# NTT123/vietTTS

Hardware: NVIDIA B200
Metric: audio_samples_per_sec (higher is better)
Workload: dtype f32 (bf16x3 split products on tcgen05, fp32 accumulate/storage)

## Files before the change

### viettts_b200/csrc/nat.cu

```cuda
#include <cooperative_groups.h>

#include "vtts_internal.cuh"

namespace cg = cooperative_groups;

namespace {

constexpr int SCAN_CTAS = 128;
constexpr int SCAN_THREADS = 256;
constexpr int UPC = 4;
constexpr int NCOL = 16;
constexpr int RG = 8;
constexpr int NSLICE = 64;
constexpr int MAX_ROWS = 128;

__device__ __forceinline__ float sigmoidf_(float x) { return 1.f / (1.f + expf(-x)); }

__host__ __device__ inline void threefry2x32(uint32_t k0, uint32_t k1, uint32_t c0, uint32_t c1, uint32_t& o0, uint32_t& o1) {
  const uint32_t ks2 = 0x1BD11BDAu ^ k0 ^ k1;
  uint32_t x0 = c0 + k0, x1 = c1 + k1;
  const int R0[4] = {13, 15, 26, 6}, R1[4] = {17, 29, 16, 24};
  const uint32_t ks[3] = {k0, k1, ks2};
#pragma unroll
  for (int blk = 0; blk < 5; ++blk) {
// ... 109 lines not shown
      acc[f][0] = fmaf(ww, x.x, acc[f][0]);
      acc[f][1] = fmaf(ww, x.y, acc[f][1]);
    }
  }
#pragma unroll
  for (int f = 0; f < UP_F; ++f) {
    const int n = f0 + f;
    if (n < nf) {
      float2 o = make_float2(acc[f][0], acc[f][1]);
      *reinterpret_cast<float2*>(out + ((size_t)b * N + n) * out_ld + tid * 2) = o;
    }
  }
}

struct Seg {
  const float* p;
  int n;
  int stride;
};

__device__ __forceinline__ float lstm_cell(const float* zs, int r, int uu, float zadd_i, float zadd_g, float zadd_f, float zadd_o, float& c) {
  const float zi = zs[r * NCOL + 0 * UPC + uu] + zadd_i;
  const float zg = zs[r * NCOL + 1 * UPC + uu] + zadd_g;
  const float zf = zs[r * NCOL + 2 * UPC + uu] + zadd_f;
  const float zo = zs[r * NCOL + 3 * UPC + uu] + zadd_o;
  const float f = sigmoidf_(zf + 1.f);
  c = f * c + sigmoidf_(zi) * tanhf(zg);
  return sigmoidf_(zo) * tanhf(c);
}

struct EncScanArgs {
  const float* zx;
  const float* whr;
  const int32_t* lengths;
  float* out;
  int B, L;
};

struct DecScanArgs {
  const float* zc0;
  const float* zc1;
  const float* w0r;
  const float* w1r;
  const float* wc;
  const float* bc;
  const float* wp2;
  const uint8_t* keep;
  uint64_t seed;
  int mode;
  float* p1;
  float* p2;
  float* h0;
  float* h1;
  unsigned int* pre_bar;
  int* err;
  float* hout;
  int B, N;
  int row_base;
  int N_total_rows;
  long long* dbg;
};

constexpr int DEC_XR = 32;
constexpr int DEC_NG = 4;
constexpr int DEC_KPAD = vc::PRENET + 2 * vc::DEC_H + 4;
constexpr int DEC_LSTM = 128, DEC_PRE = 16;
constexpr int DEC_CTAS = DEC_LSTM + DEC_PRE;

__device__ __forceinline__ void dec_fetch(float* xs, int pitch, int koff, const float* p, int n, int stride, int nr) {
  const int n4 = n >> 2;
  const int total = nr * n4;
  for (int e0 = threadIdx.x; e0 < total; e0 += SCAN_THREADS * 8) {
    float4 v[8];
#pragma unroll
    for (int u = 0; u < 8; ++u) {
      const int e = e0 + u * SCAN_THREADS;
      v[u] = make_float4(0.f, 0.f, 0.f, 0.f);
      if (e < total && p) {
        const int r = e / n4, i4 = (e - r * n4) * 4;
        v[u] = __ldcg(reinterpret_cast<const float4*>(p + (size_t)r * stride + i4));
      }
    }
#pragma unroll
    for (int u = 0; u < 8; ++u) {
      const int e = e0 + u * SCAN_THREADS;
      if (e < total) {
        const int r = e / n4, i4 = (e - r * n4) * 4;
        *reinterpret_cast<float4*>(xs + (size_t)r * pitch + koff + i4) = v[u];
      }
    }
  }
}

__device__ __forceinline__ void dec_fetch_async(float* xs, int pitch, int koff, const float* p, int n, int stride, int nr) {
  const int n4 = n >> 2;
  const int total = nr * n4;
  for (int e = threadIdx.x; e < total; e += SCAN_THREADS) {
    const int r = e / n4, i4 = (e - r * n4) * 4;
    const uint32_t dst = (uint32_t)__cvta_generic_to_shared(xs + (size_t)r * pitch + koff + i4);
    asm volatile("cp.async.cg.shared.global [%0], [%1], 16;" ::"r"(dst), "l"(p + (size_t)r * stride + i4) : "memory");
  }
  asm volatile("cp.async.commit_group;" ::: "memory");
}
template <int N>
__device__ __forceinline__ void cp_async_wait() { asm volatile("cp.async.wait_group %0;" ::"n"(N) : "memory"); }

__device__ __forceinline__ float4 warp_reduce_rows(float (&acc)[RG][4], int lane) {
  const bool b4 = lane & 16, b3 = lane & 8, b2 = lane & 4;
  float a4[4][4];
#pragma unroll
  for (int r = 0; r < 4; ++r)
#pragma unroll
    for (int c = 0; c < 4; ++c) {
      const float send = b4 ? acc[r][c] : acc[r + 4][c];
      const float keep = b4 ? acc[r + 4][c] : acc[r][c];
      a4[r][c] = keep + __shfl_xor_sync(0xffffffffu, send, 16);
    }
  float a2[2][4];
#pragma unroll
  for (int r = 0; r < 2; ++r)
#pragma unroll
    for (int c = 0; c < 4; ++c) {
      const float send = b3 ? a4[r][c] : a4[r + 2][c];
      const float keep = b3 ? a4[r + 2][c] : a4[r][c];
      a2[r][c] = keep + __shfl_xor_sync(0xffffffffu, send, 8);
    }
  float a1[4];
#pragma unroll
  for (int c = 0; c < 4; ++c) {
    const float send = b2 ? a2[0][c] : a2[1][c];
    const float keep = b2 ? a2[1][c] : a2[0][c];
    a1[c] = keep + __shfl_xor_sync(0xffffffffu, send, 4);
  }
  return make_float4(a1[0], a1[1], a1[2], a1[3]);
}

template <int SL, int PITCH = DEC_KPAD>
__device__ __forceinline__ void dec_matmul(const float* __restrict__ xs, const float (&w)[SL][4], int ngroups, float* part, float* zout,
                                           const float* zadd) {
  const int tid = threadIdx.x, lane = tid & 31, warp = tid >> 5;
  const int ks = tid >> 2;
  for (int g = 0; g < ngroups; ++g) {
    float acc[RG][4];
#pragma unroll
    for (int r = 0; r < RG; ++r) acc[r][0] = acc[r][1] = acc[r][2] = acc[r][3] = 0.f;
// ... 165 lines not shown
        acc[i][4] = fmaf(x, wb.x, acc[i][4]); acc[i][5] = fmaf(x, wb.y, acc[i][5]);
        acc[i][6] = fmaf(x, wb.z, acc[i][6]); acc[i][7] = fmaf(x, wb.w, acc[i][7]);
      }
    }
  }
  const bool b4 = lane & 16, b3 = lane & 8, b2 = lane & 4;
  float a4[4][8];
#pragma unroll
  for (int i = 0; i < 4; ++i)
#pragma unroll
    for (int c = 0; c < 8; ++c) {
      const float send = b4 ? acc[i][c] : acc[i + 4][c];
      const float keep = b4 ? acc[i + 4][c] : acc[i][c];
      a4[i][c] = keep + __shfl_xor_sync(0xffffffffu, send, 16);
    }
  float a2[2][8];
#pragma unroll
  for (int i = 0; i < 2; ++i)
#pragma unroll
    for (int c = 0; c < 8; ++c) {
      const float send = b3 ? a4[i][c] : a4[i + 2][c];
      const float keep = b3 ? a4[i + 2][c] : a4[i][c];
      a2[i][c] = keep + __shfl_xor_sync(0xffffffffu, send, 8);
    }
  float a1[8];
#pragma unroll
  for (int c = 0; c < 8; ++c) {
    const float send = b2 ? a2[0][c] : a2[1][c];
    const float keep = b2 ? a2[1][c] : a2[0][c];
    a1[c] = keep + __shfl_xor_sync(0xffffffffu, send, 4);
  }
  const int row = rg + 4 * ((lane >> 2) & 7);
  float* pw = part + ((size_t)warp * 32 + row) * 8;
  *reinterpret_cast<float4*>(pw) = make_float4(a1[0], a1[1], a1[2], a1[3]);
  *reinterpret_cast<float4*>(pw + 4) = make_float4(a1[4], a1[5], a1[6], a1[7]);
  __syncthreads();
  {
    float sum = 0.f;
#pragma unroll
    for (int wv = 0; wv < SCAN_THREADS / 32; ++wv) sum += part[(size_t)wv * 256 + tid];
    outv[tid] = sum;
  }
  __syncthreads();
}

__device__ __forceinline__ void pre_load_w8(float* wsm, const float* g, int K, int SL, int ld, int c0) {
  for (int e = threadIdx.x; e < K * 2; e += SCAN_THREADS) {
    const int k = e >> 1, h = (e & 1) * 4;
    const float4 v = __ldg(reinterpret_cast<const float4*>(g + (size_t)k * ld + c0 + h));
    *reinterpret_cast<float4*>(wsm + (size_t)(k + k / SL) * 8 + h) = v;
  }
}

__device__ __forceinline__ void prenet_barrier(unsigned int* counter, unsigned int target, int* err) {
  __syncthreads();
  if (threadIdx.x == 0) {
    __threadfence();
    atomicAdd(counter, 1u);
    const long long t0 = clock64();
    unsigned int v;
    do {
      asm volatile("ld.acquire.gpu.global.u32 %0, [%1];" : "=r"(v) : "l"(counter) : "memory");
      if (v < target && clock64() - t0 > 4000000000LL) {
        if (err) *err = 77;
        __threadfence_system();
        asm volatile("trap;");
      }
    } while (v < target);
  }
  __syncthreads();
}

__global__ void __launch_bounds__(SCAN_THREADS, 1) decoder_scan_kernel(const DecScanArgs a) {
  cg::grid_group grid = cg::this_grid();
  extern __shared__ __align__(16) float sm[];
  constexpr int H = vc::DEC_H, K0 = vc::PRENET + H, K1 = vc::PRENET + 2 * H;
  const int c = blockIdx.x, tid = threadIdx.x;
  const int B = a.B, N = a.N;
  long long tm[8] = {0, 0, 0, 0, 0, 0, 0, 0};
  long long tq = clock64();
#define DEC_MARK(i) { const long long tn = clock64(); tm[i] += tn - tq; tq = tn; }

  if (c < DEC_LSTM) {
    float* xs = sm;
    float* part = xs + DEC_XR * DEC_KPAD;
    float* zs = part + 8 * DEC_XR * NCOL;
    float* zp0 = zs + DEC_XR * NCOL;
    float* zp1 = zp0 + DEC_NG * DEC_XR * NCOL;
    float* cst = zp1 + DEC_NG * DEC_XR * NCOL;
    const int ks = tid >> 2, cgp = tid & 3;
    constexpr int SLP = vc::PRENET / NSLICE, SLH = H / NSLICE;
    float w0p[SLP][4], w0h[SLH][4], w1p[SLP][4], w1h0[SLH][4], w1h1[SLH][4];
    {
      auto ld = [&](float (&dst)[4], const float* base, int row) {
        const float4 v = __ldg(reinterpret_cast<const float4*>(base + (size_t)row * NCOL + cgp * 4));
        dst[0] = v.x; dst[1] = v.y; dst[2] = v.z; dst[3] = v.w;
      };
      const float* g0 = a.w0r + (size_t)c * K0 * NCOL;
      const float* g1 = a.w1r + (size_t)c * K1 * NCOL;
#pragma unroll
      for (int i = 0; i < SLP; ++i) { ld(w0p[i], g0, ks * SLP + i); ld(w1p[i], g1, ks * SLP + i); }
#pragma unroll
      for (int i = 0; i < SLH; ++i) {
        ld(w0h[i], g0, vc::PRENET + ks * SLH + i);
        ld(w1h0[i], g1, vc::PRENET + ks * SLH + i);
        ld(w1h1[i], g1, vc::PRENET + H + ks * SLH + i);
      }
    }
    for (int e = tid; e < DEC_NG * 2 * DEC_XR * UPC; e += SCAN_THREADS) cst[e] = 0.f;
    for (int e = tid; e < DEC_NG * 2 * DEC_XR * NCOL; e += SCAN_THREADS) zp0[e] = 0.f;
    for (int e = tid; e < DEC_XR * DEC_KPAD; e += SCAN_THREADS) xs[e] = 0.f;
    __syncthreads();
    const int NG = (B + DEC_XR - 1) / DEC_XR;
    for (int t = 0; t < N; ++t) {
      if (t > 0) {
        for (int rg = 0; rg < NG; ++rg) {
          const int r0 = rg * DEC_XR, nb = min(DEC_XR, B - r0), ngroups = (nb + RG - 1) / RG;
          if (NG > 1) dec_fetch(xs, DEC_KPAD, vc::PRENET, a.h0 + ((size_t)((t - 1) & 1) * B + r0) * H, H, H, nb);
          dec_fetch(xs, DEC_KPAD, vc::PRENET + H, a.h1 + ((size_t)((t - 1) & 1) * B + r0) * H, H, H, nb);
          if (NG > 1) __syncthreads();
          dec_matmul<SLH>(xs + vc::PRENET, w0h, ngroups, part, zp0 + rg * DEC_XR * NCOL, nullptr);
          dec_matmul<SLH>(xs + vc::PRENET + H, w1h1, ngroups, part, zp1 + rg * DEC_XR * NCOL, nullptr);
        }
      }
      DEC_MARK(0)
      DEC_MARK(1)
      DEC_MARK(2)
      grid.sync();
      DEC_MARK(3)
      for (int rg = 0; rg < NG; ++rg) {
        const int r0 = rg * DEC_XR, nb = min(DEC_XR, B - r0), ngroups = (nb + RG - 1) / RG;
        dec_fetch(xs, DEC_KPAD, 0, a.p2 + (size_t)r0 * vc::PRENET, vc::PRENET, vc::PRENET, nb);
        __syncthreads();
        dec_matmul<SLP>(xs, w0p, ngroups, part, zs, zp0 + rg * DEC_XR * NCOL);
        if (tid < nb * UPC) {
          const int r = tid / UPC, uu = tid % UPC, rb = r0 + r;
          const float* zc = a.zc0 + ((size_t)rb * N + t) * (4 * H) + c * UPC + uu;
          float* cs = cst + (size_t)rg * 2 * DEC_XR * UPC;
          float cc = cs[r * UPC + uu];
          const float h = lstm_cell(zs, r, uu, __ldg(zc), __ldg(zc + H), __ldg(zc + 2 * H), __ldg(zc + 3 * H), cc);
          cs[r * UPC + uu] = cc;
          a.h0[((size_t)(t & 1) * B + rb) * H + c * UPC + uu] = h;
          a.hout[((size_t)rb * N + t) * 2 * H + c * UPC + uu] = h;
        }
        if (NG > 1) __syncthreads();
      }
      DEC_MARK(4)
      grid.sync();
      DEC_MARK(5)
      for (int rg = 0; rg < NG; ++rg) {
        const int r0 = rg * DEC_XR, nb = min(DEC_XR, B - r0), ngroups = (nb + RG - 1) / RG;
        if (NG > 1) dec_fetch(xs, DEC_KPAD, 0, a.p2 + (size_t)r0 * vc::PRENET, vc::PRENET, vc::PRENET, nb);
        dec_fetch(xs, DEC_KPAD, vc::PRENET, a.h0 + ((size_t)(t & 1) * B + r0) * H, H, H, nb);
        __syncthreads();
        dec_matmul2<SLP, SLH>(xs, w1p, xs + vc::PRENET, w1h0, ngroups, part, zs, zp1 + rg * DEC_XR * NCOL);
        if (tid < nb * UPC) {
          const int r = tid / UPC, uu = tid % UPC, rb = r0 + r;
          const float* zc = a.zc1 + ((size_t)rb * N + t) * (4 * H) + c * UPC + uu;
          float* cs = cst + (size_t)rg * 2 * DEC_XR * UPC;
          float cc = cs[(DEC_XR + r) * UPC + uu];
          const float h = lstm_cell(zs, r, uu, __ldg(zc), __ldg(zc + H), __ldg(zc + 2 * H), __ldg(zc + 3 * H), cc);
          cs[(DEC_XR + r) * UPC + uu] = cc;
          a.h1[((size_t)(t & 1) * B + rb) * H + c * UPC + uu] = h;
          a.hout[((size_t)rb * N + t) * 2 * H + H + c * UPC + uu] = h;
        }
        __syncthreads();
      }
      DEC_MARK(6)
      grid.sync();
      DEC_MARK(7)
    }
  } else if (c < DEC_LSTM + DEC_PRE) {
    const int q = c - DEC_LSTM;
    constexpr int XP = H + 4;
    constexpr int WCB = (2 * H + 2 * H / 8) * 8;
    constexpr int W2B = (vc::PRENET + NSLICE) * 8;
    float* xs = sm;
    float* wcs = xs + 32 * XP;
    float* w2s = wcs + 2 * WCB;
    float* part = w2s + 2 * W2B;
    float* outv = part + 8 * 256;
    float* pp1 = outv + 256;
    for (int hf = 0; hf < 2; ++hf) {
      pre_load_w8(wcs + (size_t)hf * WCB, a.wc + (size_t)q * 2 * H * 16, 2 * H, 8, 16, hf * 8);
      pre_load_w8(w2s + (size_t)hf * W2B, a.wp2 + (size_t)q * vc::PRENET * 16, vc::PRENET, 4, 16, hf * 8);
    }
    for (int e = tid; e < 32 * XP; e += SCAN_THREADS) xs[e] = 0.f;
    for (int e = tid; e < DEC_NG * 512; e += SCAN_THREADS) pp1[e] = 0.f;
    __syncthreads();
    const int orow = tid >> 3, ocol = tid & 7;
    constexpr int H1OFF = (H + H / 8) * 8;
    const int NG = (B + DEC_XR - 1) / DEC_XR;
    for (int t = 0; t < N; ++t) {
      if (t > 0) {
        for (int rg = 0; rg < NG; ++rg) {
          const int r0 = rg * DEC_XR, nb = min(DEC_XR, B - r0);
          if (NG > 1) __syncthreads();
          dec_fetch(xs, XP, 0, a.h1 + ((size_t)((t - 1) & 1) * B + r0) * H, H, H, nb);
          __syncthreads();
#pragma unroll 1
          for (int hf = 0; hf < 2; ++hf) {
            pre_gemm8<8>(xs, XP, wcs + (size_t)hf * WCB + H1OFF, part, outv);
            if (orow < nb) {
              const int u = q * 16 + hf * 8 + ocol;
              const float v = fmaxf(outv[tid] + pp1[rg * 512 + hf * 256 + tid] + __ldg(a.bc + u), 0.f);
              a.p1[(size_t)(r0 + orow) * vc::PRENET + u] = v * keep_scale(a.mode, a.keep, a.seed, a.row_base + r0 + orow, t, N, 0, u);
            }
          }
        }
      } else {
        for (int e = tid; e < B * 16; e += SCAN_THREADS) a.p1[(size_t)(e >> 4) * vc::PRENET + q * 16 + (e & 15)] = 0.f;
      }
      DEC_MARK(0)
      prenet_barrier(a.pre_bar, (unsigned)DEC_PRE * (unsigned)(t + 1), a.err);
      DEC_MARK(1)
      for (int rg = 0; rg < NG; ++rg) {
        const int r0 = rg * DEC_XR, nb = min(DEC_XR, B - r0);
        if (NG > 1) __syncthreads();
        dec_fetch(xs, XP, 0, a.p1 + (size_t)r0 * vc::PRENET, vc::PRENET, vc::PRENET, nb);
        __syncthreads();
#pragma unroll 1
        for (int hf = 0; hf < 2; ++hf) {
          pre_gemm8<4>(xs, XP, w2s + (size_t)hf * W2B, part, outv);
          if (orow < nb) {
            const int u = q * 16 + hf * 8 + ocol;
            const float v = fmaxf(outv[tid], 0.f);
            a.p2[(size_t)(r0 + orow) * vc::PRENET + u] = v * keep_scale(a.mode, a.keep, a.seed, a.row_base + r0 + orow, t, N, 1, u);
          }
        }
      }
      DEC_MARK(2)
      grid.sync();
      DEC_MARK(3)
      grid.sync();
      DEC_MARK(5)
      for (int rg = 0; rg < NG; ++rg) {
        const int r0 = rg * DEC_XR, nb = min(DEC_XR, B - r0);
        __syncthreads();
        dec_fetch(xs, XP, 0, a.h0 + ((size_t)(t & 1) * B + r0) * H, H, H, nb);
        __syncthreads();
#pragma unroll 1
        for (int hf = 0; hf < 2; ++hf) {
          pre_gemm8<8>(xs, XP, wcs + (size_t)hf * WCB, part, outv);
          pp1[rg * 512 + hf * 256 + tid] = outv[tid];
        }
      }
      __syncthreads();
      DEC_MARK(6)
      grid.sync();
      DEC_MARK(7)
    }
  }
#undef DEC_MARK
  if (a.dbg && tid == 0)
    for (int i = 0; i < 8; ++i) a.dbg[(size_t)blockIdx.x * 16 + i] = tm[i];
}

__global__ void precompose_kernel(const float* __restrict__ wo, const float* __restrict__ bo, const float* __restrict__ w1,
                                  float* __restrict__ wc, float* __restrict__ bc) {
  const int o = threadIdx.x;
  const int i = blockIdx.x;
  double s = 0.0;
  if (i < 2 * vc::DEC_H) {
    for (int m = 0; m < vc::MEL; ++m) s += (double)wo[(size_t)i * vc::MEL + m] * (double)w1[(size_t)m * vc::PRENET + o];
    wc[(size_t)i * vc::PRENET + o] = (float)s;
  } else {
    for (int m = 0; m < vc::MEL; ++m) s += (double)bo[m] * (double)w1[(size_t)m * vc::PRENET + o];
    bc[o] = (float)s;
  }
}

struct TfScanArgs {
  const float* zc0;
  const float* zc1;
  const float* w0r;
  const float* w1r;
  const uint8_t* zone;
  uint64_t seed;
  int mode;
  float* h0s;
  float* h1s;
  float* hout;
  int B, N;
  int row_base;
};

constexpr int TF_PITCH = 3 * vc::DEC_H + 4;

__device__ __forceinline__ bool zone_keep(int mode, const uint8_t* zone, uint64_t seed, int b, int t, int N, int which, int unit) {
  if (mode == VTTS_DROPOUT_OFF) return false;
  if (mode == VTTS_DROPOUT_MASK) return zone[(((size_t)b * N + t) * 4 + which) * vc::DEC_H + unit] != 0;
  uint32_t o0, o1;
  (void)N;
  threefry2x32((uint32_t)seed, (uint32_t)(seed >> 32), (uint32_t)t, ((uint32_t)b << 12) | (uint32_t)(2 * vc::PRENET + which * vc::DEC_H + unit), o0, o1);
  return o0 < 429496730u;
}

__global__ void __launch_bounds__(SCAN_THREADS, 1) decoder_tf_scan_kernel(const TfScanArgs a) {
  cg::grid_group grid = cg::this_grid();
  extern __shared__ __align__(16) float sm[];
  constexpr int H = vc::DEC_H, K0 = vc::PRENET + H, K1 = vc::PRENET + 2 * H, SLH = H / NSLICE;
  const int c = blockIdx.x, tid = threadIdx.x;
  const int B = a.B, N = a.N;
// ... 38 lines not shown
      if (tid < B * UPC) {
        const int r = tid / UPC, uu = tid % UPC, u = c * UPC + uu;
        const float* zc = a.zc0 + ((size_t)r * N + s) * (4 * H) + u;
        const float c_prev = cst[r * UPC + uu];
        float cc = c_prev;
        const float h = lstm_cell(zs, r, uu, __ldg(zc), __ldg(zc + H), __ldg(zc + 2 * H), __ldg(zc + 3 * H), cc);
        const bool kh = zone_keep(a.mode, a.zone, a.seed, a.row_base + r, s, N, 0, u);
        const bool kc = zone_keep(a.mode, a.zone, a.seed, a.row_base + r, s, N, 1, u);
        a.hout[((size_t)r * N + s) * 2 * H + u] = h;
        a.h0s[((size_t)(s & 1) * B + r) * H + u] = kh ? xs[(size_t)r * TF_PITCH + u] : h;
        cst[r * UPC + uu] = kc ? c_prev : cc;
      }
    }
    cp_async_wait<0>();
    if (s >= 1) {
      const int t = s - 1;
      __syncthreads();
      dec_matmul2<SLH, SLH, TF_PITCH>(xs + H, w1h0, xs + 2 * H, w1h1, ngroups, part, zs, nullptr);
      if (tid < B * UPC) {
        const int r = tid / UPC, uu = tid % UPC, u = c * UPC + uu;
        const float* zc = a.zc1 + ((size_t)r * N + t) * (4 * H) + u;
        const float c_prev = cst[(DEC_XR + r) * UPC + uu];
        float cc = c_prev;
        const float h = lstm_cell(zs, r, uu, __ldg(zc), __ldg(zc + H), __ldg(zc + 2 * H), __ldg(zc + 3 * H), cc);
        const bool kh = zone_keep(a.mode, a.zone, a.seed, a.row_base + r, t, N, 2, u);
        const bool kc = zone_keep(a.mode, a.zone, a.seed, a.row_base + r, t, N, 3, u);
        a.hout[((size_t)r * N + t) * 2 * H + H + u] = h;
        a.h1s[((size_t)(t & 1) * B + r) * H + u] = kh ? xs[(size_t)r * TF_PITCH + 2 * H + u] : h;
        cst[(DEC_XR + r) * UPC + uu] = kc ? c_prev : cc;
      }
    }
    __syncthreads();
    grid.sync();
  }
}

__global__ void prenet_act_kernel(const float* __restrict__ x, const uint8_t* __restrict__ keep, uint64_t seed, int mode, int layer,
                                  int B, int N, float* __restrict__ out, int out_ld) {
  const size_t total = (size_t)B * N * vc::PRENET;
  for (size_t i = blockIdx.x * (size_t)blockDim.x + threadIdx.x; i < total; i += (size_t)gridDim.x * blockDim.x) {
    const int u = (int)(i % vc::PRENET);
    const size_t row = i / vc::PRENET;
    const int b = (int)(row / N), t = (int)(row % N);
    out[row * out_ld + u] = fmaxf(x[i], 0.f) * keep_scale(mode, keep, seed, b, t, N, layer, u);
  }
}

constexpr size_t tf_scan_smem() { return ((size_t)DEC_XR * TF_PITCH + 8 * DEC_XR * NCOL + DEC_XR * NCOL + 2 * DEC_XR * UPC) * 4; }

constexpr size_t enc_scan_smem() {
  return ((size_t)32 * (vc::ENC_D + 4) + 8 * DEC_XR * NCOL + DEC_XR * NCOL + MAX_ROWS * UPC) * 4;
}
constexpr size_t dec_scan_smem() {
  constexpr size_t lstm = (size_t)DEC_XR * DEC_KPAD + 8 * DEC_XR * NCOL + DEC_XR * NCOL + DEC_NG * (2 * DEC_XR * NCOL + 2 * DEC_XR * UPC);
  constexpr size_t pre = (size_t)32 * (vc::DEC_H + 4) + 2 * (2 * vc::DEC_H + 2 * vc::DEC_H / 8) * 8 + 2 * (vc::PRENET + NSLICE) * 8 + 8 * 256 + 256 + DEC_NG * 512;
  return (lstm > pre ? lstm : pre) * 4;
}

enum {
  D_ENC_BNINV0 = 0, D_ENC_BNINV1, D_ENC_BNINV2,
  D_POST_BNINV0, D_POST_BNINV1, D_POST_BNINV2, D_POST_BNINV3,
  D_ENC_WHR,
  D_DEC_W0R,
  D_DEC_W1R,
  D_DEC_WC,
  D_DEC_WCFULL,
  D_DEC_BC,
  D_DEC_WP2,
  D_ZERO,
  D_COUNT
};

enum { WP_ENC = 0, WP_ENCH = 3, WP_DECH = 11, WP_POST0 = 27, WP_POST1 = 29, WP_POST2 = 31, WP_POST3 = 33, WP_POST4 = 35, WP_PROJ = 36,
       WP_TF_L0 = 37, WP_TF_L1 = 45, WP_PRE1 = 53, WP_PRE2 = 54, WP_COUNT = 55 };

}

struct EncWeights {
  const float* embed;
  const float* conv_w[3];
  const float* conv_b[3];
  const float* bn_off[3];
  const float* bn_mean[3];
  const float* bn_inv[3];
  const float *lf_w, *lf_b, *lb_w, *lb_b;
  const float* whr;
  void* const* wpk_conv;
  void* const* wpk_hoist;
};

static int run_token_encoder(vtts_ctx* ctx, const EncWeights& w, const int32_t* tokens, const int32_t* lengths, int B, int L,
                             float* e0, float* e1, float* zx, float* enc, cudaStream_t st) {
  const size_t BL = (size_t)B * L;
  embed_kernel<<<(unsigned)((BL + 3) / 4), 256, 0, st>>>(tokens, w.embed, e0, (int)BL);
  ctx->launches++;
  VTTS_CUDA(cudaGetLastError());
  ConvLaunch Lc;
  float* cur = e0;
  float* nxt = e1;
  for (int i = 0; i < 3; ++i) {
    memset(&Lc, 0, sizeof(Lc));
    Lc.nprob = 1; Lc.Cin = 256; Lc.Cout = 256; Lc.B = B; Lc.T_rows = L; Lc.rows_out = L;
    Lc.len = lengths; Lc.len_mul = 1; Lc.pre_mode = 0; Lc.pre_slope = 1.f; Lc.post_act = 2;
    Lc.p[0] = ConvProb{cur, nullptr, nullptr, w.conv_w[i], w.conv_b[i], nullptr, w.bn_mean[i], w.bn_inv[i], w.bn_off[i], nxt, 3, 1, -1, 1, 0};
    int rc = vtts_conv_dispatch(ctx, Lc, w.wpk_conv + i, st);
    if (rc) return rc;
    float* tmp = cur; cur = nxt; nxt = tmp;
  }
  memset(&Lc, 0, sizeof(Lc));
  Lc.nprob = 2; Lc.Cin = 256; Lc.Cout = 1024; Lc.B = 1; Lc.T_rows = (int)BL; Lc.rows_out = (int)BL;
// ... 79 lines not shown
  const float* pin = melpre;
  float* pout = q0;
  int cin = 80;
  for (int i = 0; i < 5; ++i) {
    const int cout = i < 4 ? 512 : 80;
    memset(&Lc, 0, sizeof(Lc));
    Lc.nprob = 1; Lc.Cin = cin; Lc.Cout = cout; Lc.B = B; Lc.T_rows = N; Lc.rows_out = N;
    Lc.len = n_frames; Lc.len_mul = 1; Lc.pre_mode = 0; Lc.pre_slope = 1.f; Lc.post_act = i < 4 ? 1 : 0;
    ConvProb p;
    memset(&p, 0, sizeof(p));
    p.x0 = pin; p.w = T[aci::POST_CONV(i, 0)]; p.bias = T[aci::POST_CONV(i, 1)];
    if (i < 4) { p.bn_mean = T[aci::POST_CONV(i, 4)]; p.bn_inv = D[D_POST_BNINV0 + i]; p.bn_off = T[aci::POST_CONV(i, 3)]; }
    if (i == 4) { p.resid = melpre; p.out = mel; } else { p.out = pout; }
    p.k = 5; p.dil = 1; p.in_off = -2; p.out_stride = 1; p.out_off = 0;
    Lc.p[0] = p;
    int rc = vtts_conv_dispatch(ctx, Lc, &ctx->ac_wpk_t[i == 0 ? WP_POST0 : (i == 1 ? WP_POST1 : (i == 2 ? WP_POST2 : (i == 3 ? WP_POST3 : WP_POST4)))], st);
    if (rc) return rc;
    pin = pout;
    pout = (pout == q0) ? q1 : q0;
    cin = cout;
  }
  return VTTS_OK;
}

int vtts_acoustic_run(vtts_ctx* ctx, const int32_t* tokens, const int32_t* lengths, const float* dur,
                      const int32_t* n_frames, const uint8_t* keep, int mode, uint64_t seed, int B, int L, int N,
                      float* mel, cudaStream_t st, void* ws_base, size_t ws_cap, size_t* ws_need) {
  const bool measure = ws_need != nullptr;
  if (!measure) {
    if (!ctx->ac_loaded) return ctx->fail(VTTS_ERR_NOT_LOADED, "acoustic weights not loaded");
    if (B < 1 || L < 1 || N < 1 || B > MAX_ROWS)
      return ctx->fail(VTTS_ERR_BAD_ARG, "acoustic: B=%d L=%d N=%d (1 <= B <= %d rows per call; the host layer chunks larger batches)", B, L, N, MAX_ROWS);
    if (mode < 0 || mode > 2) return ctx->fail(VTTS_ERR_BAD_ARG, "acoustic: dropout_mode %d", mode);
    if (mode == VTTS_DROPOUT_MASK && !keep) return ctx->fail(VTTS_ERR_BAD_ARG, "acoustic: dropout_mode MASK needs keep_mask");
    if (ctx->sm_count < DEC_CTAS) return ctx->fail(VTTS_ERR_NO_DEVICE, "scan kernels need %d SMs, device has %d", DEC_CTAS, ctx->sm_count);
  }
  Arena ar(ws_base, ws_cap, measure);
  const size_t BL = (size_t)B * L, BN = (size_t)B * N;
  float* e0 = ar.take<float>(BL * 256);
  float* e1 = ar.take<float>(BL * 256);
  float* zx = ar.take<float>(2 * BL * 1024);
  float* enc = ar.take<float>(BL * 512);
  float* cond = ar.take<float>(BN * 512);
  float* zc0 = ar.take<float>(BN * 2048);
  float* zc1 = ar.take<float>(BN * 2048);
  float* melpre = ar.take<float>(BN * 80);
  float* q0 = ar.take<float>(BN * 512);
  float* q1 = ar.take<float>(BN * 512);
  float* p1 = ar.take<float>((size_t)B * 256);
  float* p2 = ar.take<float>((size_t)B * 256);
  float* hout = ar.take<float>(BN * 1024);
  float* h0 = ar.take<float>((size_t)2 * MAX_ROWS * 512);
  float* h1 = ar.take<float>((size_t)2 * MAX_ROWS * 512);
  unsigned int* pre_bar = ar.take<unsigned int>(64);
  if (measure) {
    *ws_need = ar.off + 256;
    return VTTS_OK;
  }
  auto& T = ctx->ac_t;
  auto& D = ctx->ac_d;
  ctx->tap_enc = enc; ctx->tap_enc_n = BL * 512;
  ctx->tap_cond = cond; ctx->tap_cond_n = BN * 512;
  ctx->tap_melpre = melpre; ctx->tap_melpre_n = BN * 80;

  VTTS_CUDA(cudaMemsetAsync(mel, 0, BN * 80 * sizeof(float), st));
  VTTS_CUDA(cudaMemsetAsync(cond, 0, BN * 512 * sizeof(float), st));
  VTTS_CUDA(cudaMemsetAsync(melpre, 0, BN * 80 * sizeof(float), st));
  ctx->sub_mark(0, st);

  {
    EncWeights ew;
    ew.embed = T[aci::EMBED];
    for (int i = 0; i < 3; ++i) {
      ew.conv_w[i] = T[aci::ENC_CONV(i, 0)]; ew.conv_b[i] = T[aci::ENC_CONV(i, 1)];
      ew.bn_off[i] = T[aci::ENC_CONV(i, 3)]; ew.bn_mean[i] = T[aci::ENC_CONV(i, 4)]; ew.bn_inv[i] = D[D_ENC_BNINV0 + i];
    }
    ew.lf_w = T[aci::ENC_LSTM_F_W]; ew.lf_b = T[aci::ENC_LSTM_F_B]; ew.lb_w = T[aci::ENC_LSTM_B_W]; ew.lb_b = T[aci::ENC_LSTM_B_B];
    ew.whr = D[D_ENC_WHR]; ew.wpk_conv = &ctx->ac_wpk_t[WP_ENC]; ew.wpk_hoist = &ctx->ac_wpk_t[WP_ENCH];
    int rc = run_token_encoder(ctx, ew, tokens, lengths, B, L, e0, e1, zx, enc, st);
    if (rc) return rc;
  }
  ctx->sub_mark(1, st);
  {
    dim3 grid((N + UP_F - 1) / UP_F, B);
    size_t smem = (size_t)(L + UP_F * L) * sizeof(float);
    if (smem > 200 * 1024) return ctx->fail(VTTS_ERR_BAD_ARG, "acoustic: L=%d too long for the upsample kernel", L);
    if (smem > 48 * 1024) VTTS_CUDA(cudaFuncSetAttribute(upsample_kernel, cudaFuncAttributeMaxDynamicSharedMemorySize, (int)smem));
    upsample_kernel<<<grid, 256, smem, st>>>(enc, dur, lengths, n_frames, L, N, cond, vc::ENC_OUT);
    ctx->launches++;
    VTTS_CUDA(cudaGetLastError());
  }
  ctx->sub_mark(2, st);
  ConvLaunch Lc;
  memset(&Lc, 0, sizeof(Lc));
  Lc.nprob = 2; Lc.Cin = 512; Lc.Cout = 2048; Lc.B = 1; Lc.T_rows = (int)BN; Lc.rows_out = (int)BN;
  Lc.pre_mode = 0; Lc.pre_slope = 1.f; Lc.post_act = 0; Lc.len_mul = 1;
  Lc.p[0] = ConvProb{cond, nullptr, nullptr, T[aci::DEC_L0_W], T[aci::DEC_L0_B], nullptr, nullptr, nullptr, nullptr, zc0, 1, 1, 0, 1, 0};
  Lc.p[1] = ConvProb{cond, nullptr, nullptr, T[aci::DEC_L1_W], T[aci::DEC_L1_B], nullptr, nullptr, nullptr, nullptr, zc1, 1, 1, 0, 1, 0};
  int rc = vtts_conv_dispatch(ctx, Lc, &ctx->ac_wpk_t[WP_DECH], st);
  if (rc) return rc;
  ctx->sub_mark(3, st);
  for (int b0 = 0; b0 < B; b0 += DEC_NG * DEC_XR) {
    const int nb = B - b0 < DEC_NG * DEC_XR ? B - b0 : DEC_NG * DEC_XR;
    DecScanArgs da;
    memset(&da, 0, sizeof(da));
    da.zc0 = zc0 + (size_t)b0 * N * 2048; da.zc1 = zc1 + (size_t)b0 * N * 2048;
    da.w0r = D[D_DEC_W0R]; da.w1r = D[D_DEC_W1R]; da.wc = D[D_DEC_WC]; da.bc = D[D_DEC_BC]; da.wp2 = D[D_DEC_WP2];
    da.keep = keep; da.seed = seed; da.mode = mode;
    da.p1 = p1; da.p2 = p2; da.h0 = h0; da.h1 = h1; da.hout = hout + (size_t)b0 * N * 1024;
    da.pre_bar = pre_bar; da.err = ctx->d_err;
    VTTS_CUDA(cudaMemsetAsync(pre_bar, 0, sizeof(unsigned int), st));
    da.B = nb; da.N = N; da.row_base = b0; da.dbg = ctx->tc_dbg_on ? ctx->d_tc_dbg : nullptr;
    void* args[] = {&da};
    VTTS_CUDA(cudaLaunchCooperativeKernel((void*)decoder_scan_kernel, dim3(DEC_CTAS), dim3(SCAN_THREADS), args, dec_scan_smem(), st));
    ctx->launches++;
  }
  ctx->sub_mark(4, st);
  memset(&Lc, 0, sizeof(Lc));
  Lc.nprob = 1; Lc.Cin = 1024; Lc.Cout = 80; Lc.B = B; Lc.T_rows = N; Lc.rows_out = N;
  Lc.len = n_frames; Lc.len_mul = 1; Lc.pre_mode = 0; Lc.pre_slope = 1.f; Lc.post_act = 0;
  Lc.p[0] = ConvProb{hout, nullptr, nullptr, T[aci::PROJ_W], T[aci::PROJ_B], nullptr, nullptr, nullptr, nullptr, melpre, 1, 1, 0, 1, 0};
  rc = vtts_conv_dispatch(ctx, Lc, &ctx->ac_wpk_t[WP_PROJ], st);
  if (rc) return rc;
  ctx->sub_mark(5, st);
  rc = run_postnet(ctx, melpre, n_frames, B, N, q0, q1, mel, st);
  if (rc) return rc;
  ctx->sub_mark(6, st);
  return VTTS_OK;
}

int vtts_acoustic_teacher_run(vtts_ctx* ctx, const int32_t* tokens, const int32_t* lengths, const float* dur,
                              const int32_t* n_frames, const float* mels_in, const uint8_t* keep, const uint8_t* zone, int mode,
                              uint64_t seed, int B, int L, int N, float* mel1, float* mel2, cudaStream_t st, void* ws_base,
                              size_t ws_cap, size_t* ws_need) {
  const bool measure = ws_need != nullptr;
  if (!measure) {
    if (!ctx->ac_loaded) return ctx->fail(VTTS_ERR_NOT_LOADED, "acoustic weights not loaded");
    if (B < 1 || L < 1 || N < 1 || B > MAX_ROWS)
      return ctx->fail(VTTS_ERR_BAD_ARG, "acoustic (teacher forced): B=%d L=%d N=%d (1 <= B <= %d rows per call)", B, L, N, MAX_ROWS);
    if (mode < 0 || mode > 2) return ctx->fail(VTTS_ERR_BAD_ARG, "acoustic (teacher forced): dropout_mode %d", mode);
    if (mode == VTTS_DROPOUT_MASK && (!keep || !zone))
      return ctx->fail(VTTS_ERR_BAD_ARG, "acoustic (teacher forced): dropout_mode MASK needs keep_mask and zone_mask");
    if (ctx->sm_count < SCAN_CTAS) return ctx->fail(VTTS_ERR_NO_DEVICE, "scan kernels need %d SMs, device has %d", SCAN_CTAS, ctx->sm_count);
  }
  Arena ar(ws_base, ws_cap, measure);
  const size_t BL = (size_t)B * L, BN = (size_t)B * N;
  constexpr int XW = vc::ENC_OUT + vc::PRENET;
  float* e0 = ar.take<float>(BL * 256);
  float* e1 = ar.take<float>(BL * 256);
  float* zx = ar.take<float>(2 * BL * 1024);
  float* enc = ar.take<float>(BL * 512);
  float* xin = ar.take<float>(BN * XW);
  float* pa = ar.take<float>(BN * 256);
  float* pb = ar.take<float>(BN * 256);
  float* zc0 = ar.take<float>(BN * 2048);
  float* zc1 = ar.take<float>(BN * 2048);
  float* hout = ar.take<float>(BN * 1024);
  float* melpre = ar.take<float>(BN * 80);
  float* q0 = ar.take<float>(BN * 512);
  float* q1 = ar.take<float>(BN * 512);
  float* h0s = ar.take<float>((size_t)2 * DEC_XR * 512);
  float* h1s = ar.take<float>((size_t)2 * DEC_XR * 512);
  if (measure) {
    *ws_need = ar.off + 256;
// ... 212 lines not shown
```

Before: 96.66 million.

## Replace decoder grid syncs with split producer/consumer counter barriers

Removes every grid.sync from the decoder scan kernel. In their place it adds separate release/acquire counters for prenet p1, p2, h0 and h1, so each CTA group waits only on the data it actually consumes. Per-step zc gate inputs are prefetched into shared memory with cp.async, hout writes are deferred until after arriving at the barrier, and dropout keep masks are precomputed one step ahead. Each thread now fetches only its own k-slice, so warp-level syncs replace block-wide ones. This adds subtle memory-ordering risk and uses more shared memory.

```diff
diff --git a/viettts_b200/csrc/nat.cu b/viettts_b200/csrc/nat.cu
--- a/viettts_b200/csrc/nat.cu
+++ b/viettts_b200/csrc/nat.cu
@@ -185,7 +185,7 @@
   float* p2;
   float* h0;
   float* h1;
-  unsigned int* pre_bar;
+  unsigned int* bar;
   int* err;
   float* hout;
   int B, N;
@@ -199,31 +199,7 @@
 constexpr int DEC_KPAD = vc::PRENET + 2 * vc::DEC_H + 4;
 constexpr int DEC_LSTM = 128, DEC_PRE = 16;
 constexpr int DEC_CTAS = DEC_LSTM + DEC_PRE;
-
-__device__ __forceinline__ void dec_fetch(float* xs, int pitch, int koff, const float* p, int n, int stride, int nr) {
-  const int n4 = n >> 2;
-  const int total = nr * n4;
-  for (int e0 = threadIdx.x; e0 < total; e0 += SCAN_THREADS * 8) {
-    float4 v[8];
-#pragma unroll
-    for (int u = 0; u < 8; ++u) {
-      const int e = e0 + u * SCAN_THREADS;
-      v[u] = make_float4(0.f, 0.f, 0.f, 0.f);
-      if (e < total && p) {
-        const int r = e / n4, i4 = (e - r * n4) * 4;
-        v[u] = __ldcg(reinterpret_cast<const float4*>(p + (size_t)r * stride + i4));
-      }
-    }
-#pragma unroll
-    for (int u = 0; u < 8; ++u) {
-      const int e = e0 + u * SCAN_THREADS;
-      if (e < total) {
-        const int r = e / n4, i4 = (e - r * n4) * 4;
-        *reinterpret_cast<float4*>(xs + (size_t)r * pitch + koff + i4) = v[u];
-      }
-    }
-  }
-}
+constexpr int DEC_BAR_P1 = 0, DEC_BAR_P2 = 16, DEC_BAR_H0 = 32, DEC_BAR_H1 = 48, DEC_BAR_WORDS = 64;
 
 __device__ __forceinline__ void dec_fetch_async(float* xs, int pitch, int koff, const float* p, int n, int stride, int nr) {
   const int n4 = n >> 2;
@@ -495,11 +471,12 @@
   }
 }
 
-__device__ __forceinline__ void prenet_barrier(unsigned int* counter, unsigned int target, int* err) {
+__device__ __forceinline__ void bar_arrive(unsigned int* counter) {
   __syncthreads();
+  if (threadIdx.x == 0) asm volatile("red.release.gpu.global.add.u32 [%0], 1;" ::"l"(counter) : "memory");
+}
+__device__ __forceinline__ void bar_wait(const unsigned int* counter, unsigned int target, int* err) {
   if (threadIdx.x == 0) {
-    __threadfence();
-    atomicAdd(counter, 1u);
     const long long t0 = clock64();
     unsigned int v;
     do {
@@ -514,8 +491,18 @@
   __syncthreads();
 }
 
+template <int SL>
+__device__ __forceinline__ void dec_fetch_slice(float* xs, int pitch, const float* p, int stride, int nr) {
+  const int ks = threadIdx.x >> 2;
+  for (int r = threadIdx.x & 3; r < nr; r += 4)
+#pragma unroll
+    for (int i = 0; i < SL; i += 4) {
+      const uint32_t dst = (uint32_t)__cvta_generic_to_shared(xs + (size_t)r * pitch + ks * SL + i);
+      asm volatile("cp.async.cg.shared.global [%0], [%1], 16;" ::"r"(dst), "l"(p + (size_t)r * stride + ks * SL + i) : "memory");
+    }
+}
+
 __global__ void __launch_bounds__(SCAN_THREADS, 1) decoder_scan_kernel(const DecScanArgs a) {
-  cg::grid_group grid = cg::this_grid();
   extern __shared__ __align__(16) float sm[];
   constexpr int H = vc::DEC_H, K0 = vc::PRENET + H, K1 = vc::PRENET + 2 * H;
   const int c = blockIdx.x, tid = threadIdx.x;
@@ -531,6 +518,8 @@
     float* zp0 = zs + DEC_XR * NCOL;
     float* zp1 = zp0 + DEC_NG * DEC_XR * NCOL;
     float* cst = zp1 + DEC_NG * DEC_XR * NCOL;
+    float* zcs = cst + DEC_NG * 2 * DEC_XR * UPC;
+    float* hsm = zcs + 2 * MAX_ROWS * NCOL;
     const int ks = tid >> 2, cgp = tid & 3;
     constexpr int SLP = vc::PRENET / NSLICE, SLH = H / NSLICE;
     float w0p[SLP][4], w0h[SLH][4], w1p[SLP][4], w1h0[SLH][4], w1h1[SLH][4];
@@ -556,62 +545,78 @@
     __syncthreads();
     const int NG = (B + DEC_XR - 1) / DEC_XR;
     for (int t = 0; t < N; ++t) {
+      for (int e = tid; e < B * 8; e += SCAN_THREADS) {
+        const int rb = e >> 3, l = (e >> 2) & 1, g = e & 3;
+        const float* src = (l ? a.zc1 : a.zc0) + ((size_t)rb * N + t) * (4 * H) + g * H + c * UPC;
+        const uint32_t dst = (uint32_t)__cvta_generic_to_shared(zcs + ((size_t)l * MAX_ROWS + rb) * NCOL + g * UPC);
+        asm volatile("cp.async.cg.shared.global [%0], [%1], 16;" ::"r"(dst), "l"(src) : "memory");
+      }
+      asm volatile("cp.async.commit_group;" ::: "memory");
       if (t > 0) {
+        bar_wait(a.bar + DEC_BAR_H1, (unsigned)DEC_LSTM * (unsigned)t, a.err);
+        DEC_MARK(7)
         for (int rg = 0; rg < NG; ++rg) {
           const int r0 = rg * DEC_XR, nb = min(DEC_XR, B - r0), ngroups = (nb + RG - 1) / RG;
-          if (NG > 1) dec_fetch(xs, DEC_KPAD, vc::PRENET, a.h0 + ((size_t)((t - 1) & 1) * B + r0) * H, H, H, nb);
-          dec_fetch(xs, DEC_KPAD, vc::PRENET + H, a.h1 + ((size_t)((t - 1) & 1) * B + r0) * H, H, H, nb);
-          if (NG > 1) __syncthreads();
+          if (NG > 1) dec_fetch_slice<SLH>(xs + vc::PRENET, DEC_KPAD, a.h0 + ((size_t)((t - 1) & 1) * B + r0) * H, H, nb);
+          dec_fetch_slice<SLH>(xs + vc::PRENET + H, DEC_KPAD, a.h1 + ((size_t)((t - 1) & 1) * B + r0) * H, H, nb);
+          asm volatile("cp.async.commit_group;" ::: "memory");
+          cp_async_wait<0>();
+          __syncwarp();
           dec_matmul<SLH>(xs + vc::PRENET, w0h, ngroups, part, zp0 + rg * DEC_XR * NCOL, nullptr);
           dec_matmul<SLH>(xs + vc::PRENET + H, w1h1, ngroups, part, zp1 + rg * DEC_XR * NCOL, nullptr);
         }
       }
       DEC_MARK(0)
-      DEC_MARK(1)
-      DEC_MARK(2)
-      grid.sync();
+      bar_wait(a.bar + DEC_BAR_P2, (unsigned)DEC_PRE * (unsigned)(t + 1), a.err);
       DEC_MARK(3)
       for (int rg = 0; rg < NG; ++rg) {
         const int r0 = rg * DEC_XR, nb = min(DEC_XR, B - r0), ngroups = (nb + RG - 1) / RG;
-        dec_fetch(xs, DEC_KPAD, 0, a.p2 + (size_t)r0 * vc::PRENET, vc::PRENET, vc::PRENET, nb);
-        __syncthreads();
+        dec_fetch_slice<SLP>(xs, DEC_KPAD, a.p2 + (size_t)r0 * vc::PRENET, vc::PRENET, nb);
+        asm volatile("cp.async.commit_group;" ::: "memory");
+        cp_async_wait<0>();
+        __syncwarp();
         dec_matmul<SLP>(xs, w0p, ngroups, part, zs, zp0 + rg * DEC_XR * NCOL);
         if (tid < nb * UPC) {
           const int r = tid / UPC, uu = tid % UPC, rb = r0 + r;
-          const float* zc = a.zc0 + ((size_t)rb * N + t) * (4 * H) + c * UPC + uu;
+          const float* zc = zcs + (size_t)rb * NCOL + uu;
           float* cs = cst + (size_t)rg * 2 * DEC_XR * UPC;
           float cc = cs[r * UPC + uu];
-          const float h = lstm_cell(zs, r, uu, __ldg(zc), __ldg(zc + H), __ldg(zc + 2 * H), __ldg(zc + 3 * H), cc);
+          const float h = lstm_cell(zs, r, uu, zc[0], zc[UPC], zc[2 * UPC], zc[3 * UPC], cc);
           cs[r * UPC + uu] = cc;
           a.h0[((size_t)(t & 1) * B + rb) * H + c * UPC + uu] = h;
-          a.hout[((size_t)rb * N + t) * 2 * H + c * UPC + uu] = h;
+          hsm[rb * UPC + uu] = h;
         }
         if (NG > 1) __syncthreads();
       }
+      bar_arrive(a.bar + DEC_BAR_H0);
+      for (int e = tid; e < B * UPC; e += SCAN_THREADS) a.hout[((size_t)(e / UPC) * N + t) * 2 * H + c * UPC + e % UPC] = hsm[e];
       DEC_MARK(4)
-      grid.sync();
+      bar_wait(a.bar + DEC_BAR_H0, (unsigned)DEC_LSTM * (unsigned)(t + 1), a.err);
       DEC_MARK(5)
       for (int rg = 0; rg < NG; ++rg) {
         const int r0 = rg * DEC_XR, nb = min(DEC_XR, B - r0), ngroups = (nb + RG - 1) / RG;
-        if (NG > 1) dec_fetch(xs, DEC_KPAD, 0, a.p2 + (size_t)r0 * vc::PRENET, vc::PRENET, vc::PRENET, nb);
-        dec_fetch(xs, DEC_KPAD, vc::PRENET, a.h0 + ((size_t)(t & 1) * B + r0) * H, H, H, nb);
-        __syncthreads();
+        if (NG > 1) dec_fetch_slice<SLP>(xs, DEC_KPAD, a.p2 + (size_t)r0 * vc::PRENET, vc::PRENET, nb);
+        dec_fetch_slice<SLH>(xs + vc::PRENET, DEC_KPAD, a.h0 + ((size_t)(t & 1) * B + r0) * H, H, nb);
+        asm volatile("cp.async.commit_group;" ::: "memory");
+        cp_async_wait<0>();
+        __syncwarp();
         dec_matmul2<SLP, SLH>(xs, w1p, xs + vc::PRENET, w1h0, ngroups, part, zs, zp1 + rg * DEC_XR * NCOL);
         if (tid < nb * UPC) {
           const int r = tid / UPC, uu = tid % UPC, rb = r0 + r;
-          const float* zc = a.zc1 + ((size_t)rb * N + t) * (4 * H) + c * UPC + uu;
+          const float* zc = zcs + ((size_t)MAX_ROWS + rb) * NCOL + uu;
           float* cs = cst + (size_t)rg * 2 * DEC_XR * UPC;
           float cc = cs[(DEC_XR + r) * UPC + uu];
-          const float h = lstm_cell(zs, r, uu, __ldg(zc), __ldg(zc + H), __ldg(zc + 2 * H), __ldg(zc + 3 * H), cc);
+          const float h = lstm_cell(zs, r, uu, zc[0], zc[UPC], zc[2 * UPC], zc[3 * UPC], cc);
           cs[(DEC_XR + r) * UPC + uu] = cc;
           a.h1[((size_t)(t & 1) * B + rb) * H + c * UPC + uu] = h;
-          a.hout[((size_t)rb * N + t) * 2 * H + H + c * UPC + uu] = h;
+          hsm[(MAX_ROWS + rb) * UPC + uu] = h;
         }
-        __syncthreads();
-      }
+        if (NG > 1) __syncthreads();
+      }
+      bar_arrive(a.bar + DEC_BAR_H1);
+      for (int e = tid; e < B * UPC; e += SCAN_THREADS)
+        a.hout[((size_t)(e / UPC) * N + t) * 2 * H + H + c * UPC + e % UPC] = hsm[MAX_ROWS * UPC + e];
       DEC_MARK(6)
-      grid.sync();
-      DEC_MARK(7)
     }
   } else if (c < DEC_LSTM + DEC_PRE) {
     const int q = c - DEC_LSTM;
@@ -624,6 +629,7 @@
     float* part = w2s + 2 * W2B;
     float* outv = part + 8 * 256;
     float* pp1 = outv + 256;
+    float* kp = pp1 + DEC_NG * 512;
     for (int hf = 0; hf < 2; ++hf) {
       pre_load_w8(wcs + (size_t)hf * WCB, a.wc + (size_t)q * 2 * H * 16, 2 * H, 8, 16, hf * 8);
       pre_load_w8(w2s + (size_t)hf * W2B, a.wp2 + (size_t)q * vc::PRENET * 16, vc::PRENET, 4, 16, hf * 8);
@@ -634,20 +640,32 @@
     const int orow = tid >> 3, ocol = tid & 7;
     constexpr int H1OFF = (H + H / 8) * 8;
     const int NG = (B + DEC_XR - 1) / DEC_XR;
+    auto draw_keeps = [&](int tt) {
+      for (int rg = 0; rg < NG; ++rg) {
+        const int r0 = rg * DEC_XR, nb = min(DEC_XR, B - r0);
+        if (orow < nb)
+#pragma unroll
+          for (int i = 0; i < 4; ++i)
+            kp[(rg * 4 + i) * 256 + tid] = keep_scale(a.mode, a.keep, a.seed, a.row_base + r0 + orow, tt, N, i >> 1, q * 16 + (i & 1) * 8 + ocol);
+      }
+    };
+    draw_keeps(0);
     for (int t = 0; t < N; ++t) {
       if (t > 0) {
+        bar_wait(a.bar + DEC_BAR_H1, (unsigned)DEC_LSTM * (unsigned)t, a.err);
+        DEC_MARK(7)
         for (int rg = 0; rg < NG; ++rg) {
           const int r0 = rg * DEC_XR, nb = min(DEC_XR, B - r0);
-          if (NG > 1) __syncthreads();
-          dec_fetch(xs, XP, 0, a.h1 + ((size_t)((t - 1) & 1) * B + r0) * H, H, H, nb);
-          __syncthreads();
+          dec_fetch_slice<8>(xs, XP, a.h1 + ((size_t)((t - 1) & 1) * B + r0) * H, H, nb);
+          asm volatile("cp.async.commit_group;" ::: "memory");
+          cp_async_wait<0>();
 #pragma unroll 1
           for (int hf = 0; hf < 2; ++hf) {
             pre_gemm8<8>(xs, XP, wcs + (size_t)hf * WCB + H1OFF, part, outv);
             if (orow < nb) {
               const int u = q * 16 + hf * 8 + ocol;
               const float v = fmaxf(outv[tid] + pp1[rg * 512 + hf * 256 + tid] + __ldg(a.bc + u), 0.f);
-              a.p1[(size_t)(r0 + orow) * vc::PRENET + u] = v * keep_scale(a.mode, a.keep, a.seed, a.row_base + r0 + orow, t, N, 0, u);
+              a.p1[(size_t)(r0 + orow) * vc::PRENET + u] = v * kp[(rg * 4 + hf) * 256 + tid];
             }
           }
         }
@@ -655,43 +673,42 @@
         for (int e = tid; e < B * 16; e += SCAN_THREADS) a.p1[(size_t)(e >> 4) * vc::PRENET + q * 16 + (e & 15)] = 0.f;
       }
       DEC_MARK(0)
-      prenet_barrier(a.pre_bar, (unsigned)DEC_PRE * (unsigned)(t + 1), a.err);
+      bar_arrive(a.bar + DEC_BAR_P1);
+      bar_wait(a.bar + DEC_BAR_P1, (unsigned)DEC_PRE * (unsigned)(t + 1), a.err);
       DEC_MARK(1)
       for (int rg = 0; rg < NG; ++rg) {
         const int r0 = rg * DEC_XR, nb = min(DEC_XR, B - r0);
-        if (NG > 1) __syncthreads();
-        dec_fetch(xs, XP, 0, a.p1 + (size_t)r0 * vc::PRENET, vc::PRENET, vc::PRENET, nb);
-        __syncthreads();
+        dec_fetch_slice<4>(xs, XP, a.p1 + (size_t)r0 * vc::PRENET, vc::PRENET, nb);
+        asm volatile("cp.async.commit_group;" ::: "memory");
+        cp_async_wait<0>();
 #pragma unroll 1
         for (int hf = 0; hf < 2; ++hf) {
           pre_gemm8<4>(xs, XP, w2s + (size_t)hf * W2B, part, outv);
           if (orow < nb) {
             const int u = q * 16 + hf * 8 + ocol;
             const float v = fmaxf(outv[tid], 0.f);
-            a.p2[(size_t)(r0 + orow) * vc::PRENET + u] = v * keep_scale(a.mode, a.keep, a.seed, a.row_base + r0 + orow, t, N, 1, u);
+            a.p2[(size_t)(r0 + orow) * vc::PRENET + u] = v * kp[(rg * 4 + 2 + hf) * 256 + tid];
           }
         }
       }
+      bar_arrive(a.bar + DEC_BAR_P2);
       DEC_MARK(2)
-      grid.sync();
+      if (t + 1 < N) draw_keeps(t + 1);
       DEC_MARK(3)
-      grid.sync();
+      bar_wait(a.bar + DEC_BAR_H0, (unsigned)DEC_LSTM * (unsigned)(t + 1), a.err);
       DEC_MARK(5)
       for (int rg = 0; rg < NG; ++rg) {
         const int r0 = rg * DEC_XR, nb = min(DEC_XR, B - r0);
-        __syncthreads();
-        dec_fetch(xs, XP, 0, a.h0 + ((size_t)(t & 1) * B + r0) * H, H, H, nb);
-        __syncthreads();
+        dec_fetch_slice<8>(xs, XP, a.h0 + ((size_t)(t & 1) * B + r0) * H, H, nb);
+        asm volatile("cp.async.commit_group;" ::: "memory");
+        cp_async_wait<0>();
 #pragma unroll 1
         for (int hf = 0; hf < 2; ++hf) {
           pre_gemm8<8>(xs, XP, wcs + (size_t)hf * WCB, part, outv);
           pp1[rg * 512 + hf * 256 + tid] = outv[tid];
         }
       }
-      __syncthreads();
       DEC_MARK(6)
-      grid.sync();
-      DEC_MARK(7)
     }
   }
 #undef DEC_MARK
@@ -836,10 +853,13 @@
   return ((size_t)32 * (vc::ENC_D + 4) + 8 * DEC_XR * NCOL + DEC_XR * NCOL + MAX_ROWS * UPC) * 4;
 }
 constexpr size_t dec_scan_smem() {
-  constexpr size_t lstm = (size_t)DEC_XR * DEC_KPAD + 8 * DEC_XR * NCOL + DEC_XR * NCOL + DEC_NG * (2 * DEC_XR * NCOL + 2 * DEC_XR * UPC);
-  constexpr size_t pre = (size_t)32 * (vc::DEC_H + 4) + 2 * (2 * vc::DEC_H + 2 * vc::DEC_H / 8) * 8 + 2 * (vc::PRENET + NSLICE) * 8 + 8 * 256 + 256 + DEC_NG * 512;
+  constexpr size_t lstm = (size_t)DEC_XR * DEC_KPAD + 8 * DEC_XR * NCOL + DEC_XR * NCOL + DEC_NG * (2 * DEC_XR * NCOL + 2 * DEC_XR * UPC) +
+                          2 * MAX_ROWS * NCOL + 2 * MAX_ROWS * UPC;
+  constexpr size_t pre = (size_t)32 * (vc::DEC_H + 4) + 2 * (2 * vc::DEC_H + 2 * vc::DEC_H / 8) * 8 + 2 * (vc::PRENET + NSLICE) * 8 + 8 * 256 + 256 +
+                         DEC_NG * 512 + DEC_NG * 4 * 256;
   return (lstm > pre ? lstm : pre) * 4;
 }
+static_assert(dec_scan_smem() <= 227 * 1024, "decoder scan: shared memory of one CTA");
 
 enum {
   D_ENC_BNINV0 = 0, D_ENC_BNINV1, D_ENC_BNINV2,
@@ -1025,7 +1045,7 @@
   float* hout = ar.take<float>(BN * 1024);
   float* h0 = ar.take<float>((size_t)2 * MAX_ROWS * 512);
   float* h1 = ar.take<float>((size_t)2 * MAX_ROWS * 512);
-  unsigned int* pre_bar = ar.take<unsigned int>(64);
+  unsigned int* dec_bar = ar.take<unsigned int>(DEC_BAR_WORDS);
   if (measure) {
     *ws_need = ar.off + 256;
     return VTTS_OK;
@@ -1081,8 +1101,8 @@
     da.w0r = D[D_DEC_W0R]; da.w1r = D[D_DEC_W1R]; da.wc = D[D_DEC_WC]; da.bc = D[D_DEC_BC]; da.wp2 = D[D_DEC_WP2];
     da.keep = keep; da.seed = seed; da.mode = mode;
     da.p1 = p1; da.p2 = p2; da.h0 = h0; da.h1 = h1; da.hout = hout + (size_t)b0 * N * 1024;
-    da.pre_bar = pre_bar; da.err = ctx->d_err;
-    VTTS_CUDA(cudaMemsetAsync(pre_bar, 0, sizeof(unsigned int), st));
+    da.bar = dec_bar; da.err = ctx->d_err;
+    VTTS_CUDA(cudaMemsetAsync(dec_bar, 0, DEC_BAR_WORDS * sizeof(unsigned int), st));
     da.B = nb; da.N = N; da.row_base = b0; da.dbg = ctx->tc_dbg_on ? ctx->d_tc_dbg : nullptr;
     void* args[] = {&da};
     VTTS_CUDA(cudaLaunchCooperativeKernel((void*)decoder_scan_kernel, dim3(DEC_CTAS), dim3(SCAN_THREADS), args, dec_scan_smem(), st));
```

After: 96.46 million (median of 6 runs). No clear change (-0.2%).
